# channable/alfred-margaret

Measured on AMD Instinct MI355X. Metric: GiB/s haystack bytes scanned (match-emitting runLower, 100k-needle automaton), higher is better.
Workload: dtype u8

## Files before the change

alfred-margaret_amd/csrc/am_kernels.hip:

```cpp
#include <hip/hip_runtime.h>

#include <atomic>
#include <cstdlib>
#include <type_traits>

#include "am_bounds.h"
#include "am_config.h"
#include "am_device.h"
#include "am_wave.h"

AM_BOUNDS_TU("am_kernels.hip")

namespace am {
namespace dev {


__global__ void k_hidx(const uint64_t* __restrict__ offsets, uint32_t n_hay, uint64_t total, uint32_t* __restrict__ hidx, uint64_t n_entries,
                       uint32_t* __restrict__ z0, uint64_t n0, uint32_t* __restrict__ z1, uint64_t n1)
{
    const uint64_t k = (uint64_t)blockIdx.x * blockDim.x + threadIdx.x;
    const uint64_t stride = (uint64_t)gridDim.x * blockDim.x;
    for (uint64_t i = k; i < n0; i += stride) z0[i] = 0u;
    for (uint64_t i = k; i < n1; i += stride) z1[i] = 0u;
    if (k >= n_entries) return;
    uint64_t p = k << kHidxShift;
    if (p > total - 1) p = total - 1;
    uint32_t lo = 0, hi = n_hay - 1;
    while (lo < hi) {
        const uint32_t mid = lo + (hi - lo + 1u) / 2u;
        if (offsets[mid] <= p) lo = mid; else hi = mid - 1u;
    }
    hidx[k] = lo;
}


constexpr int kSfThreads = 1024;
constexpr int kSfWaves = kSfThreads / 64;
constexpr int kSfLightThreads = 256;
constexpr uint64_t kSfLightChunks = 16;
constexpr int kSfQ1 = 128;
constexpr int kSfQ2 = 256;
constexpr uint32_t kSfMaxUnitChunks = 64;
constexpr uint32_t kSfWqIters = 2;
constexpr uint32_t kSfEpochChunks = 16;
constexpr int kSfStage = 1056;
constexpr uint32_t kSfMaskBytes = kBloomMasks * 4u;

template <bool IC, int MODE, int ILP, int LW, bool SHORT, bool DBG, int NT = kSfThreads, bool CHILDREN = false>
__global__ __launch_bounds__(NT) void k_sf(SfView s, BatchView b, ScanOut o, uint64_t n_chunks)
{
    constexpr int kSfThreads = NT, kSfWaves = NT / 64;
    constexpr bool kFlagMode = MODE == kModeAny || MODE == kModeIds;
    constexpr bool CH = CHILDREN, children = CHILDREN;
    constexpr uint32_t kEpoch = kFlagMode ? 4u : CH ? 8u : kSfEpochChunks;
    extern __shared__ __attribute__((aligned(16))) uint32_t lds[];
    const uint32_t words = 1u << s.bloom_log2_words;
    uint32_t* masks = lds;
    uint32_t* bloom = lds + kBloomMasks;
    uint8_t* stage_all = reinterpret_cast<uint8_t*>(bloom + words);
    uint16_t* q1_all = reinterpret_cast<uint16_t*>(stage_all + kSfWaves * kSfStage);
    uint16_t* q2_all = q1_all + kSfWaves * kSfQ1;

    for (uint32_t i = threadIdx.x; i < kBloomMasks; i += kSfThreads) masks[i] = bloom_mask_entry(i);
    for (uint32_t i = threadIdx.x; i < words; i += kSfThreads) bloom[i] = s.scan_bloom[i];
    __syncthreads();

    const uint32_t lane = threadIdx.x & 63u, wave = __builtin_amdgcn_readfirstlane(threadIdx.x >> 6);
    const uint32_t stage = kSfMaskBytes + 4u * words + wave * (uint32_t)kSfStage;
    const uint32_t q1 = kSfMaskBytes + 4u * words + (uint32_t)kSfWaves * kSfStage + wave * (uint32_t)(kSfQ1 * 2);
    const uint32_t q2 = kSfMaskBytes + 4u * words + (uint32_t)kSfWaves * (kSfStage + kSfQ1 * 2) + wave * (uint32_t)(kSfQ2 * 2);
    const uint32_t wq_cap = o.wq_cap;
    const uint32_t wq = kSfMaskBytes + 4u * words + (uint32_t)kSfWaves * (kSfStage + kSfQ1 * 2 + kSfQ2 * 2) + wave * (wq_cap * 64u);
    uint32_t wq_n = 0;
    (void)stage_all; (void)q1_all; (void)q2_all;
    const uint64_t n_waves = (uint64_t)gridDim.x * kSfWaves;
    const uint32_t log2_words = s.bloom_log2_words, tiers = s.tiers & ~kSfKeyFold;
    const uint32_t UC = o.unit_chunks;
    const uint64_t n_units = (n_chunks + UC - 1) / UC;
    uint64_t nval = 0;
    uint32_t q2_head = 0, q2_tail = 0;
    uint64_t unit_base_chunk = 0, epoch_base_chunk = 0;
    uint32_t unit_count = 0, unit_slots = 0, cur_block = kNone, first_block = kNone, grant_next = 0, grant_left = 0;
    bool pool_ok = true;

    const bool timing = DBG && o.dbg != nullptr;
    uint64_t t_filter = 0, t_compact = 0, t_probe = 0, t_resolve = 0, t_probe_pre = 0, t_mark = 0;
    uint64_t dbg_iters[8] = {0, 0, 0, 0, 0, 0, 0, 0};
    uint64_t t_r0 = 0, t_r1 = 0, t_r2 = 0, t_r3 = 0, n_batches = 0, n_cand = 0, n_probes = 0, n_defer = 0, n_found = 0;
    auto tick = [&](uint64_t& acc) { if (timing) { const uint64_t now = __builtin_amdgcn_s_memtime(); acc += now - t_mark; t_mark = now; } };

    uint32_t cnt_hay = kNone; uint64_t cnt_val = 0;
    auto flush_count = [&]() {
        if (cnt_hay != kNone && cnt_val && lane == 0) atomicAdd(reinterpret_cast<unsigned long long*>(o.hay_counts + cnt_hay), (unsigned long long)cnt_val);
        cnt_val = 0;
    };
    auto add_counts = [&](bool found, uint32_t hay, uint32_t vlen) {
        if (found) nval += vlen;
        const uint64_t fm = __ballot(found);
        if (!o.hay_counts || !fm) return;
        const uint32_t h0 = __shfl(hay, __ffsll((unsigned long long)fm) - 1, 64);
        if (__ballot(found && hay != h0) == 0) {
            const uint64_t sum = wave_sum_u64(found ? (uint64_t)vlen : 0ull);
            if (h0 != cnt_hay) { flush_count(); cnt_hay = h0; }
            cnt_val += sum;
        } else if (found) atomicAdd(reinterpret_cast<unsigned long long*>(o.hay_counts + hay), (unsigned long long)vlen);
    };
    auto walk_parked = [&]() {
        const uint32_t n = wq_n < 64u ? wq_n : 64u, base = wq_n - n;
        wq_n = base;
        const bool valid = lane < n;
        const uint32_t e = wq + (base + (valid ? lane : 0u)) * 64u;
        const u32x4_n a0 = *reinterpret_cast<const lds_u32x4_t*>((uintptr_t)e), a1 = *reinterpret_cast<const lds_u32x4_t*>((uintptr_t)(e + 16u)),
                      a2 = *reinterpret_cast<const lds_u32x4_t*>((uintptr_t)(e + 32u)), a3 = *reinterpret_cast<const lds_u32x4_t*>((uintptr_t)(e + 48u));
        uint64_t gpos[1] = {((uint64_t)a0.y << 32) | a0.x};
        uint32_t avail[1] = {a0.z}, depth[1] = {a1.x}, best_state[1] = {a1.y}, best_vlen[1] = {a1.z}, w2[1] = {a1.w}, node[1] = {kNone};
        const uint32_t slot = a0.w, hay = a3.z, prior = a1.y;
        SfNode rec[1] = {SfNode{0, 0, a2.x, a2.y, {a2.z, a2.w, a3.x, a3.y}}};
        bool go[1] = {valid}, have_rec[1] = {true};
        wave_lds_fence();
        uint32_t sel[1] = {a3.w};
        sf_resolve_walk<IC, 1>(s, b.text, gpos, avail, w2, go, node, rec, have_rec, depth, best_state, best_vlen, nullptr, 0xFFFFFFFFu, nullptr, sel);
        if (SHORT) {
            const bool vv[1] = {valid && !best_state[0]};
            uint32_t w[1] = {0}, dummy = 0;
            if (vv[0]) { load_suffix8(b.text, gpos[0], w[0], dummy); if (IC) w[0] = fold_dword(w[0]); }
            sf_resolve_short<1>(s, vv, avail, w, best_state, best_vlen);
        }
        const bool found = valid && best_state[0] != 0;
        if (timing) n_found += (uint32_t)__popcll(__ballot(found && prior == 0u));
        if (MODE == kModeCount) add_counts(found, hay, best_vlen[0]);
        else if (MODE == kModeEmit) {
            if (found && best_state[0] != prior && pool_ok) { AM_BOUNDS(slot < (uint64_t)o.n_blocks * kPoolBlock); o.pool[slot].state = best_state[0] - 1u; }
            unit_count += (uint32_t)__popcll(__ballot(found && prior == 0u));
        } else if (MODE == kModeAny && found) atomicOr(reinterpret_cast<uint32_t*>(o.flags) + (hay >> 2), 1u << (8u * (hay & 3u)));
    };

    constexpr int RN = 1;
    auto resolve_batch = [&](uint32_t nb, bool drain) {
        __builtin_amdgcn_s_setprio(3);
        if (timing) { const uint64_t now = __builtin_amdgcn_s_memtime(); t_r0 += now - t_mark; t_mark = now; n_batches++; }
        uint64_t gpos[RN];
        uint32_t w2[RN], avail[RN], best_state[RN], best_vlen[RN], depth[RN], hay[RN], slot[RN], sel[RN];
        SfNode rec[RN];
        bool parked[RN];
        uint64_t pm[RN];
#pragma unroll
        for (int k = 0; k < RN; k++) {
            gpos[k] = 0; w2[k] = avail[k] = best_state[k] = best_vlen[k] = depth[k] = hay[k] = slot[k] = 0;
            rec[k] = SfNode{0, 0, 0, 0, {0, 0, 0, 0}}; parked[k] = false; pm[k] = 0; sel[k] = kSelUnknown;
        }
        if (nb) {
            bool valid[RN];
            uint32_t hint[RN], hlo[RN], hhi[RN];
            uint64_t end_pos[RN];
#pragma unroll
            for (int k = 0; k < RN; k++) {
                valid[k] = 64u * k + lane < nb;
                const uint32_t item = valid[k] ? lds_read_u16(q2 + 2u * ((q2_head + 64u * k + lane) % kSfQ2)) : 0u;
                gpos[k] = (epoch_base_chunk + ((item >> 12) & (kEpoch - 1u))) * kSfChunk + (item & 1023u);
                hint[k] = ((item >> 10) & 3u) | ((CH && children) ? (item >> 13) & 4u : 0u);
                hlo[k] = hhi[k] = 0; end_pos[k] = 0;
                if (valid[k]) { hlo[k] = b.hidx[gpos[k] >> kHidxShift]; hhi[k] = b.hidx[(gpos[k] >> kHidxShift) + 1]; }
            }
            auto locate = [&]() {
#pragma unroll
                for (int k = 0; k < RN; k++) {
                    hay[k] = hlo[k];
                    uint64_t start = valid[k] ? b.offsets[hlo[k]] : 0;
                    if (valid[k] && hlo[k] != hhi[k]) { hay[k] = find_haystack(b, gpos[k]); start = b.offsets[hay[k]]; }
                    end_pos[k] = valid[k] ? gpos[k] - start + 1 : 0;
                }
            };
            uint32_t w[RN], node[RN], t16[RN][4];
            bool go[RN], have_rec[RN], found[RN];
            sf_resolve_head<IC, RN>(s, b.text, gpos, end_pos, valid, hint, locate, w, w2, avail, best_state, best_vlen, depth, go, node, rec, have_rec, t16, timing ? dbg_iters : nullptr);
            sf_resolve_walk<IC, RN>(s, b.text, gpos, avail, w2, go, node, rec, have_rec, depth, best_state, best_vlen, timing ? dbg_iters : nullptr, wq_cap ? o.wq_iters : 0xFFFFFFFFu, t16, sel);
#pragma unroll
            for (int k = 0; k < RN; k++) parked[k] = go[k] && valid[k];
            if (SHORT) {
                bool vv[RN];
#pragma unroll
                for (int k = 0; k < RN; k++) vv[k] = valid[k] && !parked[k];
                sf_resolve_short<RN>(s, vv, avail, w, best_state, best_vlen);
            }
#pragma unroll
            for (int k = 0; k < RN; k++) {
                found[k] = valid[k] && best_state[k] != 0;
                if (timing) n_found += (uint32_t)__popcll(__ballot(found[k]));
            }
            if (MODE == kModeCount) {
#pragma unroll
                for (int k = 0; k < RN; k++) add_counts(found[k] && !parked[k], hay[k], best_vlen[k]);
            } else if (MODE == kModeEmit && RN == 1) {
                const uint64_t take_mask = __ballot(found[0] || parked[0]);
                const uint32_t F = (uint32_t)__popcll(take_mask);
                if (F) {
                    const uint32_t r = unit_slots & (kPoolBlock - 1u);
                    const bool need_new = r == 0u || r + F > kPoolBlock;
                    uint32_t new_block = kNone;
                    if (need_new) {
                        if (grant_left == 0) {
                            uint32_t g = 0;
                            if (lane == 0) g = atomicAdd(o.pool_ctrl, kSfBlockGrant);
                            grant_next = __builtin_amdgcn_readfirstlane(g);
                            grant_left = kSfBlockGrant;
                        }
                        const uint32_t id = grant_next++;
                        grant_left--;
                        if (id >= o.n_blocks) { pool_ok = false; if (lane == 0) o.pool_ctrl[1] = 1u; }
                        else {
                            new_block = id;
                            if (lane == 0) { o.block_next[id] = kNone; if (cur_block != kNone) o.block_next[cur_block] = id; }
                            if (first_block == kNone) first_block = id;
                        }
                    }
                    if ((found[0] || parked[0]) && pool_ok) {
                        const uint32_t p = r + (uint32_t)__popcll(take_mask & ((1ull << lane) - 1ull));
                        slot[0] = (r != 0u && p < kPoolBlock) ? cur_block * kPoolBlock + p : new_block * kPoolBlock + (r != 0u ? p - kPoolBlock : p);
                        AM_BOUNDS(slot[0] < (uint64_t)o.n_blocks * kPoolBlock && hay[0] < b.n_hay);
                        o.pool[slot[0]] = Record{end_pos[0], hay[0], found[0] ? best_state[0] - 1u : kNone};
                    }
                    if (need_new && pool_ok) cur_block = new_block;
                    unit_slots += F;
                    unit_count += (uint32_t)__popcll(__ballot(found[0]));
                }
            } else if (MODE == kModeEmit) {
                uint64_t take[RN]; uint32_t before[RN], F = 0, n_found_recs = 0;
#pragma unroll
                for (int k = 0; k < RN; k++) {
                    take[k] = __ballot(found[k] || parked[k]); before[k] = F; F += (uint32_t)__popcll(take[k]);
                    n_found_recs += (uint32_t)__popcll(__ballot(found[k]));
                }
                if (F) {
                    const uint32_t s0 = unit_slots, have = (s0 + kPoolBlock - 1u) / kPoolBlock;
                    const uint32_t n_new = (s0 + F + kPoolBlock - 1u) / kPoolBlock - have;
                    const uint32_t prev_block = cur_block;
                    uint32_t ids[RN + 1];
#pragma unroll
                    for (int t = 0; t < RN + 1; t++) {
                        ids[t] = kNone;
                        if ((uint32_t)t < n_new) {
                            if (grant_left == 0) {
                                uint32_t g = 0;
                                if (lane == 0) g = atomicAdd(o.pool_ctrl, kSfBlockGrant);
                                grant_next = __builtin_amdgcn_readfirstlane(g);
                                grant_left = kSfBlockGrant;
                            }
                            const uint32_t id = grant_next++;
                            grant_left--;
                            if (id >= o.n_blocks) { pool_ok = false; if (lane == 0) o.pool_ctrl[1] = 1u; }
                            else if (pool_ok) {
                                ids[t] = id;
                                if (lane == 0) { o.block_next[id] = kNone; if (cur_block != kNone) o.block_next[cur_block] = id; }
                                if (first_block == kNone) first_block = id;
                                cur_block = id;
                            }
                        }
                    }
#pragma unroll
                    for (int k = 0; k < RN; k++) {
                        if ((found[k] || parked[k]) && pool_ok) {
                            const uint32_t si = s0 + before[k] + (uint32_t)__popcll(take[k] & ((1ull << lane) - 1ull));
                            const uint32_t q = si / kPoolBlock;
                            uint32_t blk = prev_block;
#pragma unroll
                            for (int t = 0; t < RN + 1; t++) if (q == have + (uint32_t)t) blk = ids[t];
                            slot[k] = blk * kPoolBlock + (si & (kPoolBlock - 1u));
                            AM_BOUNDS(slot[k] < (uint64_t)o.n_blocks * kPoolBlock && hay[k] < b.n_hay);
                            o.pool[slot[k]] = Record{end_pos[k], hay[k], found[k] ? best_state[k] - 1u : kNone};
                        }
                    }
                    unit_slots += F;
                    unit_count += n_found_recs;
                }
            } else if (MODE == kModeAny) {
#pragma unroll
                for (int k = 0; k < RN; k++) {
                    const uint64_t fm = __ballot(found[k]);
                    if (fm) {
                        const uint32_t h0 = __shfl(hay[k], __ffsll((unsigned long long)fm) - 1, 64);
                        const bool same = __ballot(found[k] && hay[k] != h0) == 0;
                        const bool mine = found[k] && (same ? lane == (uint32_t)__ffsll((unsigned long long)fm) - 1u : true);
                        if (mine) {
                            uint32_t* word = reinterpret_cast<uint32_t*>(o.flags) + (hay[k] >> 2);
                            const uint32_t bit = 1u << (8u * (hay[k] & 3u));
                            if (!(__atomic_load_n(word, __ATOMIC_RELAXED) & bit)) atomicOr(word, bit);
                        }
                    }
                }
            } else {
#pragma unroll
                for (int k = 0; k < RN; k++) {
                    if (found[k]) {
                        const uint32_t st = best_state[k] - 1u;
                        uint32_t* row = o.ids_bits + (uint64_t)hay[k] * o.ids_words;
                        for (uint64_t v = o.ids_vals_off[st], ve = o.ids_vals_off[st + 1]; v < ve; v++) {
                            const uint32_t id = o.ids_vals[v];
                            if (id >= o.ids_n) continue;
                            const uint32_t bit = 1u << (id & 31u);
                            if (row[id >> 5] & bit) continue;
                            if (!(atomicOr(row + (id >> 5), bit) & bit) && atomicSub(o.ids_missing + hay[k], 1u) == 1u)
                                atomicOr(reinterpret_cast<uint32_t*>(o.flags) + (hay[k] >> 2), 1u << (8u * (hay[k] & 3u)));
                        }
                    }
                }
            }
#pragma unroll
            for (int k = 0; k < RN; k++) pm[k] = __ballot(parked[k]);
        }
        uint64_t pm_any = 0;
#pragma unroll
        for (int k = 0; k < RN; k++) pm_any |= pm[k];
        if (pm_any || (drain && wq_n)) {
            int next_k = 0;
            for (;;) {
#pragma unroll
                for (int k = 0; k < RN; k++) {
                    if (next_k == k) {
                        const uint32_t n_park = (uint32_t)__popcll(pm[k]);
                        if (wq_n + n_park <= wq_cap) {
                            if (parked[k]) {
                                const uint32_t e = wq + (wq_n + (uint32_t)__popcll(pm[k] & ((1ull << lane) - 1ull))) * 64u;
                                AM_BOUNDS(e + 64u <= wq + wq_cap * 64u);
                                lds_write_u32x4(e, make_uint4((uint32_t)gpos[k], (uint32_t)(gpos[k] >> 32), avail[k], slot[k]));
                                lds_write_u32x4(e + 16u, make_uint4(depth[k], best_state[k], best_vlen[k], w2[k]));
                                lds_write_u32x4(e + 32u, make_uint4(rec[k].z, rec[k].w, rec[k].label[0], rec[k].label[1]));
                                lds_write_u32x4(e + 48u, make_uint4(rec[k].label[2], rec[k].label[3], hay[k], sel[k]));
                            }
                            wq_n += n_park;
                            wave_lds_fence();
                            next_k = k + 1;
                        }
                    }
                }
                if (next_k == RN && (drain ? wq_n == 0u : wq_n < 64u)) break;
                walk_parked();
                wave_lds_fence();
            }
        }
        if (timing) { const uint64_t now = __builtin_amdgcn_s_memtime(); t_r3 += now - t_mark; t_mark = now; }
        q2_head += nb;
        __builtin_amdgcn_s_setprio(2);
    };

    u32x2 p_a[2], p_b[2];
    uint32_t p_e[2] = {0, 0}, p_pos[2] = {0, 0};
    uint32_t p_k5[2] = {0, 0}, p_e5[2] = {0, 0};
    uint32_t p_ci = 0;
    bool pending = false, p_two = false;
    p_a[0] = p_a[1] = p_b[0] = p_b[1] = u32x2{0, 0};
    auto consume_round = [&]() {
        auto park = [&](bool defer, uint32_t hint, uint32_t pos) {
            const uint64_t m = __ballot(defer);
            AM_BOUNDS(q2_tail - q2_head + (uint32_t)__popcll(m) <= (uint32_t)kSfQ2);
            if (defer) lds_write_u16(q2 + 2u * ((q2_tail + (uint32_t)__popcll(m & ((1ull << lane) - 1ull))) % kSfQ2), (p_ci << 12) | ((hint & 3u) << 10) | (pos & 1023u) | (CH ? (hint & 4u) << 13 : 0u));
            q2_tail += (uint32_t)__popcll(m);
            if (timing) n_defer += (uint32_t)__popcll(m);
        };
        if (ILP == 2 || p_two) {
            bool valid[2], defer[2];
            uint32_t hint[2];
#pragma unroll
            for (int k = 0; k < 2; k++) valid[k] = (p_pos[k] & 0x8000u) != 0;
            sf_probe_decide<2>(s, p_a, p_b, p_e, valid, defer, hint);
            if (CH && children) {
                bool heavy[2];
                sf_probe_heavy<2>(s, p_a, p_b, p_e, defer, heavy);
                if (wave_any(heavy[0] || heavy[1])) sf_probe_children<2>(s, p_k5, p_e5, heavy, defer, hint);
            }
            park(defer[0], hint[0], p_pos[0]);
            park(defer[1], hint[1], p_pos[1]);
        } else {
            const u32x2 a1[1] = {p_a[0]}, b1[1] = {p_b[0]};
            const uint32_t e1[1] = {p_e[0]};
            const bool valid[1] = {(p_pos[0] & 0x8000u) != 0};
            bool defer[1]; uint32_t hint[1];
            sf_probe_decide<1>(s, a1, b1, e1, valid, defer, hint);
            if (CH && children) {
                bool heavy[1];
                sf_probe_heavy<1>(s, a1, b1, e1, defer, heavy);
                if (wave_any(heavy[0])) { const uint32_t k5[1] = {p_k5[0]}, e5[1] = {p_e5[0]}; sf_probe_children<1>(s, k5, e5, heavy, defer, hint); }
            }
            park(defer[0], hint[0], p_pos[0]);
        }
        pending = false;
    };

    auto fetch = [&](uint64_t cc, uint4& v) {
        const uint64_t p = cc * kSfChunk + lane * 16u;
        v = make_uint4(0, 0, 0, 0);
        if (cc < n_chunks && p < b.total) {
            typedef uint32_t u32x4_native __attribute__((ext_vector_type(4)));
            const u32x4_native* src = reinterpret_cast<const u32x4_native*>(b.text + p);
            const u32x4_native t = *src;
            v = make_uint4(t.x, t.y, t.z, t.w);
        }
    };
    auto fetch_before = [&](uint64_t cc, uint32_t& c3, uint32_t& c4) {
        uint2 t = make_uint2(0, 0);
        if (cc < n_chunks && cc > 0) {
            t = *reinterpret_cast<const uint2*>(b.text + cc * kSfChunk - 8);
            t.x = (uint32_t)__builtin_amdgcn_readfirstlane((int)t.x); t.y = (uint32_t)__builtin_amdgcn_readfirstlane((int)t.y);
        }
        c3 = IC ? fold_dword(t.x) : t.x; c4 = IC ? fold_dword(t.y) : t.y;
    };
    const uint64_t t_begin = timing ? __builtin_amdgcn_s_memtime() : 0;
    if (timing) t_mark = t_begin;
    uint64_t u = (uint64_t)blockIdx.x * kSfWaves + wave;
    uint64_t hs0 = 1, he0 = 0; uint32_t hay0 = 0;
    uint4 cur_v; uint32_t carry3, carry4;
    fetch(u * UC, cur_v);
    fetch_before(u * UC, carry3, carry4);
    asm volatile("" : "+v"(cur_v.x), "+v"(cur_v.y), "+v"(cur_v.z), "+v"(cur_v.w));

    uint32_t any_word = 0, any_hay = kNone, flagged_hay = kNone;

    uint64_t u_next = u;
    for (; u < n_units; u = u_next) {
        u_next = u + n_waves;
        if (o.next_unit && !kFlagMode) {
            uint32_t ticket = 0;
            if (lane == 0) ticket = atomicAdd(o.next_unit, 1u);
            u_next = n_waves + (uint32_t)__builtin_amdgcn_readfirstlane((int)ticket);
        }
        unit_base_chunk = u * UC;
        unit_count = 0; unit_slots = 0; cur_block = kNone; first_block = kNone;
        const uint32_t n_in_unit = (uint32_t)(unit_base_chunk + UC <= n_chunks ? UC : n_chunks - unit_base_chunk);
        if (kFlagMode && flagged_hay != kNone && hay0 == flagged_hay) {
            const uint64_t ub = unit_base_chunk * kSfChunk, ue0 = ub + (uint64_t)n_in_unit * kSfChunk, ue = ue0 < b.total ? ue0 : b.total;
            if (ub >= hs0 && he0 >= b.total) break;
            if (ub >= hs0 && ue <= he0) {
                fetch(u_next * UC, cur_v);
                fetch_before(u_next * UC, carry3, carry4);
                asm volatile("" : "+v"(cur_v.x), "+v"(cur_v.y), "+v"(cur_v.z), "+v"(cur_v.w));
                continue;
            }
        }
        bool jumped = false;
        for (uint32_t ci = 0; ci < n_in_unit; ci++) {
            const uint64_t c = unit_base_chunk + ci;
            if ((ci & (kEpoch - 1u)) == 0 && !jumped) epoch_base_chunk = c;
            uint4 next_v = make_uint4(0, 0, 0, 0);
            uint32_t next_c3 = 0, next_c4 = 0;
            const bool last_of_unit = ci + 1 >= n_in_unit;
            if (kFlagMode && any_hay != kNone) {
                const uint32_t seen = (uint32_t)__builtin_amdgcn_readfirstlane((int)any_word);
                if (((seen >> (8u * (any_hay & 3u))) & 0xFFu) != 0u) flagged_hay = any_hay;
                any_hay = kNone;
            }
            if (kFlagMode && last_of_unit) {
                if (flagged_hay != kNone && flagged_hay == hay0 && he0 >= b.total && unit_base_chunk * kSfChunk >= hs0) u_next = n_units;
                else if (o.next_unit) {
                    uint32_t ticket = 0;
                    if (lane == 0) ticket = atomicAdd(o.next_unit, 1u);
                    u_next = n_waves + (uint32_t)__builtin_amdgcn_readfirstlane((int)ticket);
                }
            }
            const bool next_skipped = kFlagMode && !last_of_unit && flagged_hay != kNone && flagged_hay == hay0 &&
                                      (c + 1) * kSfChunk >= hs0 && (c + 2) * kSfChunk <= he0;
            if (!next_skipped)
            fetch(!last_of_unit ? c + 1 : u_next * UC, next_v);
            if (last_of_unit) fetch_before(u_next * UC, next_c3, next_c4);

            const uint64_t c0 = c * kSfChunk;
            const uint64_t p0 = c0 + lane * 16u;
            if (c0 >= he0 || c0 < hs0) {
                hay0 = (uint32_t)__builtin_amdgcn_readfirstlane((int)b.hidx[c0 >> kHidxShift]);
                hs0 = uniform_u64(b.offsets[hay0]); he0 = uniform_u64(b.offsets[hay0 + 1]);
            }
            const bool single = (c0 + kSfChunk < b.total ? c0 + kSfChunk : b.total) <= he0;
            bool skip = false;
            if (kFlagMode) {
                skip = single && flagged_hay == hay0;
                if (skip && ci + 2 < n_in_unit) {
                    const uint64_t ue0 = (unit_base_chunk + n_in_unit) * kSfChunk;
                    if ((ue0 < b.total ? ue0 : b.total) <= he0) { ci = n_in_unit - 2u; jumped = true; }
                }
                if (!skip && (ci & 7u) == 0u) {
                    any_word = __hip_atomic_load(reinterpret_cast<const uint32_t*>(o.flags) + (hay0 >> 2), __ATOMIC_RELAXED, __HIP_MEMORY_SCOPE_AGENT);
                    any_hay = hay0;
                }
            }

            uint32_t d1 = cur_v.x, d2 = cur_v.y, d3 = cur_v.z, d4 = cur_v.w;
            if (IC) { d1 = fold_dword(d1); d2 = fold_dword(d2); d3 = fold_dword(d3); d4 = fold_dword(d4); }
            const uint32_t d0 = (uint32_t)__builtin_amdgcn_update_dpp((int)carry4, (int)d4, 0x138, 0xf, 0xf, false);
            const uint32_t f[5] = {bloom_key(d0, IC), bloom_key(d1, IC), bloom_key(d2, IC), bloom_key(d3, IC), bloom_key(d4, IC)};
            lds_write_u32x4(stage + 16u + lane * 16u, make_uint4(d1, d2, d3, d4));
            if (lane == 0) lds_write_u32x2(stage + 8u, make_uint2(carry3, carry4));
            if (!last_of_unit) {
                next_c3 = (uint32_t)__builtin_amdgcn_readlane((int)d3, 63);
                next_c4 = (uint32_t)__builtin_amdgcn_readlane((int)d4, 63);
            }
            __builtin_amdgcn_s_setprio(0);
            uint32_t cand = 0;
            if (!kFlagMode || !skip) {
                uint32_t h[16], v[16], m[16];
                const uint32_t sh_word = 32u - log2_words;
#pragma unroll
                for (int k = 0; k < 16; k++) {
                    const int j = k >> 2, sh = k & 3;
                    const uint32_t w = sh == 3 ? f[j + 1] : __builtin_amdgcn_alignbyte(f[j + 1], f[j], sh + 1);
                    h[k] = w * kBloomMul;
                }
#pragma unroll
                for (int k = 15; k >= 0; k--) {
                    if (LW) v[k] = lds_read_u32(kSfMaskBytes + ((h[k] >> (30 - LW)) & (((1u << LW) - 1u) << 2)));
                    else v[k] = lds_read_u32(kSfMaskBytes + ((h[k] >> sh_word) << 2));
                    m[k] = lds_read_u32(h[k] & ((kBloomMasks - 1u) << 2));
                }
                __builtin_amdgcn_sched_barrier(0);
#pragma unroll
                for (int k = 15; k >= 0; k--) {
                    const uint32_t mr = rotr32(m[k], scan_rot(h[k]));
                    cand = shift_in_eq(cand, v[k] & mr, mr);
                }
            }
            if (SHORT && (!kFlagMode || !skip)) {
#pragma unroll
                for (int k = 0; k < 16; k++) {
                    const int j = k >> 2, sh = k & 3;
                    const uint32_t w = sh == 3 ? f[j + 1] : __builtin_amdgcn_alignbyte(f[j + 1], f[j], sh + 1);
                    if (sf_filter_short<true>(bloom, log2_words, tiers, w, masks)) cand |= 1u << k;
                }
            }
            __builtin_amdgcn_s_setprio(2);
            if (p0 + 16 > b.total) cand &= p0 < b.total ? (1u << (uint32_t)(b.total - p0)) - 1u : 0u;
            if (timing) { asm volatile("" :: "v"(cand)); tick(t_filter); }

            for (bool first = true;; first = false) {
                const uint32_t n = __popc(cand);
                const uint32_t incl = wave_inclusive_sum(n, lane);
                const uint32_t total = wave_last_lane(incl);
                if (total == 0 && !(first && pending)) break;
                uint32_t idx = incl - n;
                while (cand && idx < (uint32_t)kSfQ1) {
                    const uint32_t k = __builtin_ctz(cand);
                    cand &= cand - 1u;
                    AM_BOUNDS(idx < (uint32_t)kSfQ1);
                    lds_write_u16(q1 + 2u * idx++, lane * 16u + k);
                }
                const uint32_t n_q1 = total < (uint32_t)kSfQ1 ? total : (uint32_t)kSfQ1;
                if (timing) n_cand += n_q1;
                wave_lds_fence();
                tick(t_compact);
                if (pending) {
                    consume_round();
                    wave_lds_fence();
                    tick(t_probe);
                    while (q2_tail - q2_head >= 64u * RN) { resolve_batch(64u * RN, false); wave_lds_fence(); }
                    tick(t_resolve);
                }
                if (n_q1) {
                    uint64_t avail[2] = {0, 0};
                    uint32_t w[2] = {0, 0}, nb[2] = {0, 0};
                    bool valid[2] = {false, false};
                    const bool two = ILP == 2 || n_q1 > 64u || o.two_always;
                    p_pos[1] = 0u;
#pragma unroll
                    for (int k = 0; k < 2; k++) {
                        if (k == 1 && !two) break;
                        const uint32_t e = 64u * k + lane;
                        valid[k] = e < n_q1;
                        const uint32_t pos = valid[k] ? lds_read_u16(q1 + 2u * e) : 0u;
                        if (CH && children) {
                            const uint32_t a = 10u + pos, sh = a & 3u;
                            const uint32_t sp = stage + (a & ~3u);
                            const uint32_t x0 = lds_read_u32(sp), x1 = lds_read_u32(sp + 4u), x2 = lds_read_u32(sp + 8u);
                            const uint32_t three = __builtin_amdgcn_alignbyte(x1, x0, sh) & 0xFFFFFFu;
                            const uint32_t nbs3 = (three >> 16) | (three & 0xFF00u) | ((three & 0xFFu) << 16);
                            nb[k] = nbs3 & 0xFFFFu;
                            w[k] = sh < 1u ? __builtin_amdgcn_alignbyte(x1, x0, 3u) : __builtin_amdgcn_alignbyte(x2, x1, sh - 1u);
                            t4_child_inputs(s, w[k], nbs3, p_k5[k], p_e5[k]);
                        } else {
                        const uint32_t a = 11u + pos, sh = a & 3u;
                        const uint32_t sp = stage + (a & ~3u);
                        const uint32_t x0 = lds_read_u32(sp), x1 = lds_read_u32(sp + 4u), x2 = lds_read_u32(sp + 8u);
                        const uint32_t two = __builtin_amdgcn_alignbyte(x1, x0, sh) & 0xFFFFu;
                        nb[k] = (two >> 8) | ((two & 0xFFu) << 8);
                        w[k] = sh < 2u ? __builtin_amdgcn_alignbyte(x1, x0, sh + 2u) : __builtin_amdgcn_alignbyte(x2, x1, sh - 2u);
                        }
                        const uint64_t gpos = c0 + pos;
                        avail[k] = gpos - hs0 + 1;
                        if (valid[k] && !single) avail[k] = gpos - b.offsets[find_haystack(b, gpos)] + 1;
                        p_pos[k] = valid[k] ? (pos | 0x8000u) : 0u;
                    }
                    if (two) sf_probe_issue<2>(s, w, nb, avail, valid, p_a, p_b, p_e);
                    else {
                        const uint32_t w1[1] = {w[0]}, nb1[1] = {nb[0]};
                        const uint64_t av1[1] = {avail[0]};
                        const bool v1[1] = {valid[0]};
                        u32x2 a1[1], b1[1]; uint32_t e1[1];
                        sf_probe_issue<1>(s, w1, nb1, av1, v1, a1, b1, e1);
                        p_a[0] = a1[0]; p_b[0] = b1[0]; p_e[0] = e1[0];
                    }
                    p_two = two;
                    p_ci = ci & (kEpoch - 1u);
                    pending = true;
                    if (timing) { n_probes++; tick(t_probe_pre); }
                }
                if (total <= (uint32_t)kSfQ1) break;
                wave_lds_fence();
            }
            cur_v = next_v; carry3 = next_c3; carry4 = next_c4;
            if ((ci & (kEpoch - 1u)) == kEpoch - 1u || last_of_unit) {
                if (pending) consume_round();
                wave_lds_fence();
                tick(t_compact);
                const bool walk_all = last_of_unit || kFlagMode;
                while (q2_tail != q2_head || (walk_all && wq_n)) {
                    const uint32_t left = q2_tail - q2_head, nb = left < 64u * RN ? left : 64u * RN;
                    resolve_batch(nb, walk_all && left == nb);
                }
                tick(t_resolve);
            }
        }
        if (MODE == kModeEmit && lane == 0) { o.unit_counts[u] = unit_count; o.unit_first[u] = first_block; o.unit_slots[u] = unit_slots; }
    }
    if (timing && lane == 0) {
        atomicAdd(reinterpret_cast<unsigned long long*>(o.dbg + 0), (unsigned long long)t_filter);
        atomicAdd(reinterpret_cast<unsigned long long*>(o.dbg + 1), (unsigned long long)t_compact);
        atomicAdd(reinterpret_cast<unsigned long long*>(o.dbg + 2), (unsigned long long)t_probe);
        atomicAdd(reinterpret_cast<unsigned long long*>(o.dbg + 3), (unsigned long long)t_resolve);
        atomicAdd(reinterpret_cast<unsigned long long*>(o.dbg + 4), 1ull);
        atomicAdd(reinterpret_cast<unsigned long long*>(o.dbg + 5), (unsigned long long)t_probe_pre);
        atomicAdd(reinterpret_cast<unsigned long long*>(o.dbg + 6), (unsigned long long)n_batches);
        atomicAdd(reinterpret_cast<unsigned long long*>(o.dbg + 7), (unsigned long long)t_r0);
        atomicAdd(reinterpret_cast<unsigned long long*>(o.dbg + 8), (unsigned long long)t_r1);
        atomicAdd(reinterpret_cast<unsigned long long*>(o.dbg + 9), (unsigned long long)t_r2);
        atomicAdd(reinterpret_cast<unsigned long long*>(o.dbg + 10), (unsigned long long)t_r3);
        for (int i = 0; i < 7; i++) atomicAdd(reinterpret_cast<unsigned long long*>(o.dbg + 16 + 2 * 8192 + i), (unsigned long long)dbg_iters[i]);
        atomicAdd(reinterpret_cast<unsigned long long*>(o.dbg + 11), (unsigned long long)n_cand);
        atomicAdd(reinterpret_cast<unsigned long long*>(o.dbg + 12), (unsigned long long)n_probes);
        atomicAdd(reinterpret_cast<unsigned long long*>(o.dbg + 13), (unsigned long long)n_defer);
        atomicAdd(reinterpret_cast<unsigned long long*>(o.dbg + 14), (unsigned long long)n_found);
        atomicMax(reinterpret_cast<unsigned long long*>(o.dbg + 15), (unsigned long long)(__builtin_amdgcn_s_memtime() - t_begin));
        const uint64_t gw = (uint64_t)blockIdx.x * kSfWaves + wave;
        if (gw < 8192) {
            uint32_t hw_id, xcc_id;
            asm volatile("s_getreg_b32 %0, hwreg(HW_REG_HW_ID)" : "=s"(hw_id));
            asm volatile("s_getreg_b32 %0, hwreg(HW_REG_XCC_ID)" : "=s"(xcc_id));
            o.dbg[16 + 2 * gw] = __builtin_amdgcn_s_memtime() - t_begin;
            o.dbg[17 + 2 * gw] = ((uint64_t)xcc_id << 32) | hw_id;
        }
    }

    if (MODE == kModeCount) {
        if (o.hay_counts) flush_count();
        nval = wave_sum_u64(nval);
        if (lane == 0 && nval) atomicAdd(reinterpret_cast<unsigned long long*>(o.total_values), (unsigned long long)nval);
    }
}

__global__ __launch_bounds__(256) void k_permute(ScanOut o, const uint64_t* __restrict__ unit_offsets, Record* __restrict__ out, uint64_t n_units)
{
    const uint64_t u = ((uint64_t)blockIdx.x * blockDim.x + threadIdx.x) >> 6;
    const uint32_t lane = threadIdx.x & 63u;
    if (u >= n_units) return;
    const uint32_t n = o.unit_slots[u];
    uint64_t at = unit_offsets[u];
    uint32_t blk = o.unit_first[u];
    const uint4* pool4 = reinterpret_cast<const uint4*>(o.pool);
    uint4* out4 = reinterpret_cast<uint4*>(out);
    for (uint32_t done = 0; done < n; done += kPoolBlock) {
        if (blk == kNone) break;
        uint4 r = make_uint4(0u, 0u, 0u, kNone);
        if (done + lane < n) r = pool4[(uint64_t)blk * kPoolBlock + lane];
        const uint64_t m = __ballot(r.w != kNone);
        if (r.w != kNone) out4[at + (uint32_t)__popcll(m & ((1ull << lane) - 1ull))] = r;
        at += (uint32_t)__popcll(m);
        blk = o.block_next[blk];
    }
}


hipError_t launch_hidx(const BatchView& b, uint32_t* hidx, uint64_t n_entries, hipStream_t st, uint32_t* z0, uint64_t n0, uint32_t* z1, uint64_t n1)
{
    const uint32_t blocks = (uint32_t)((n_entries + 255) / 256);
    hipLaunchKernelGGL(k_hidx, dim3(blocks), dim3(256), 0, st, b.offsets, b.n_hay, b.total, hidx, n_entries, z0, n0, z1, n1);
    return hipGetLastError();
}

uint64_t sf_chunks(const BatchView& b) { return (b.total + kSfChunk - 1) / kSfChunk; }

uint32_t sf_unit_chunks(const BatchView& b, int n_cu)
{
    const uint64_t n_chunks = sf_chunks(b), waves = (uint64_t)(n_cu > 0 ? n_cu : 1) * kSfWaves;
    const uint64_t per_wave = (n_chunks + waves - 1) / waves;
    const uint64_t k = (per_wave + kSfMaxUnitChunks - 1) / kSfMaxUnitChunks;
    if (k >= 4) return kSfMaxUnitChunks;
    const uint64_t uc = k <= 1 ? per_wave : (n_chunks + waves * k - 1) / (waves * k);
    return (uint32_t)(uc < 1 ? 1 : uc);
}

hipError_t launch_permute(const ScanOut& o, const uint64_t* unit_offsets, Record* out, uint64_t n_units, hipStream_t st)
{
    if (n_units == 0) return hipSuccess;
    const uint64_t blocks = (n_units * 64 + 255) / 256;
    hipLaunchKernelGGL(k_permute, dim3((uint32_t)blocks), dim3(256), 0, st, o, unit_offsets, out, n_units);
    return hipGetLastError();
}
uint64_t ac_units(const AcView& a, const BatchView& b) { return (b.total + a.chunk - 1) / a.chunk; }

static size_t sf_lds_bytes_w(const SfView& s, int waves) { return kSfMaskBytes + ((size_t)4 << s.bloom_log2_words) + (size_t)waves * (kSfStage + kSfQ1 * sizeof(uint16_t) + kSfQ2 * sizeof(uint16_t)); }
static uint32_t sf_wq_cap(const SfView& s, int waves)
{
    const size_t base = sf_lds_bytes_w(s, waves), limit = 160 * 1024;
    if (base >= limit) return 0;
    size_t cap = (limit - base) / ((size_t)waves * 64);
    if (cap > 128) cap = 128;
    return cap >= 64 ? (uint32_t)cap : 0u;
}
size_t sf_lds_bytes(const SfView& s) { return sf_lds_bytes_w(s, kSfWaves); }

constexpr uint32_t kSfVariantValid = 1u, kSfVariantIc = 2u, kSfVariantModeShift = 2, kSfVariantIlpShift = 4, kSfVariantShort = 1u << 6, kSfVariantDbg = 1u << 7,
                   kSfVariantLight = 1u << 8, kSfVariantChildren = 1u << 9, kSfVariantLwShift = 16;
static std::atomic<uint32_t> g_sf_last_variant{0};
uint32_t take_sf_last_variant() { return g_sf_last_variant.exchange(0, std::memory_order_relaxed); }

template <bool IC, int MODE, int ILP, int LW, bool SHORT, bool DBG = false, int NT = kSfThreads, bool CHILDREN = false>
static hipError_t launch_sf_v(const SfView& s, const BatchView& b, const ScanOut& o, int n_cu, hipStream_t st)
{
    constexpr int waves_per_wg = NT / 64;
    constexpr bool kFlagMode = MODE == kModeAny || MODE == kModeIds;
    const uint32_t wq_cap = kFlagMode ? 0u : sf_wq_cap(s, waves_per_wg);
    const size_t lds = sf_lds_bytes_w(s, waves_per_wg) + (size_t)waves_per_wg * wq_cap * 64;
    static bool attr_set = false;
    if (!attr_set) {
        if (hipFuncSetAttribute(reinterpret_cast<const void*>(&k_sf<IC, MODE, ILP, LW, SHORT, DBG, NT, CHILDREN>), hipFuncAttributeMaxDynamicSharedMemorySize, 160 * 1024) != hipSuccess)
            (void)hipGetLastError();
        attr_set = true;
    }
    const uint64_t n_chunks = sf_chunks(b);
    const int per_cu = NT == kSfThreads ? (lds <= 80 * 1024 ? 2 : 1) : 8;
    uint64_t blocks = (uint64_t)n_cu * per_cu;
    const uint64_t n_units = (n_chunks + o.unit_chunks - 1) / o.unit_chunks;
    const uint64_t need = (n_units + waves_per_wg - 1) / waves_per_wg;
    if (blocks > need) blocks = need;
    if (blocks == 0) return hipSuccess;
    g_sf_last_variant.store(kSfVariantValid | (IC ? kSfVariantIc : 0u) | ((uint32_t)MODE << kSfVariantModeShift) | ((uint32_t)ILP << kSfVariantIlpShift) | (SHORT ? kSfVariantShort : 0u) |
                            (DBG ? kSfVariantDbg : 0u) | (NT == kSfLightThreads ? kSfVariantLight : 0u) | (CHILDREN ? kSfVariantChildren : 0u) | ((uint32_t)LW << kSfVariantLwShift),
                            std::memory_order_relaxed);
    ScanOut oo = o;
    oo.wq_cap = wq_cap;
    oo.wq_iters = kSfWqIters;
    if (n_units <= blocks * waves_per_wg) oo.next_unit = nullptr;
    hipLaunchKernelGGL((k_sf<IC, MODE, ILP, LW, SHORT, DBG, NT, CHILDREN>), dim3((uint32_t)blocks), dim3(NT), lds, st, s, b, oo, n_chunks);
    return hipGetLastError();
}

static uint64_t* g_sf_dbg = nullptr;
hipError_t read_sf_wave_records(uint64_t* out, size_t n_waves)
{
    if (!g_sf_dbg) return hipErrorInvalidValue;
    if (n_waves == 0) { hipError_t e = hipMemcpy(out, g_sf_dbg + 16 + 2 * 8192, 64, hipMemcpyDeviceToHost); if (e == hipSuccess) e = hipMemset(g_sf_dbg + 16 + 2 * 8192, 0, 64); return e; }
    return hipMemcpy(out, g_sf_dbg + 16, 16 * (n_waves < 8192 ? n_waves : 8192), hipMemcpyDeviceToHost);
}

hipError_t read_sf_phase_cycles(uint64_t* out5)
{
    for (int i = 0; i < 16; i++) out5[i] = 0;
    if (!g_sf_dbg) return hipSuccess;
    hipError_t e = hipMemcpy(out5, g_sf_dbg, 128, hipMemcpyDeviceToHost);
    if (e == hipSuccess) e = hipMemset(g_sf_dbg, 0, 128);
    return e;
}

template <bool IC, int MODE>
static hipError_t launch_sf_t(const SfView& s, const BatchView& b, const ScanOut& o, int n_cu, hipStream_t st)
{
    const bool lw15 = s.bloom_log2_words == 15;
    constexpr bool kFlagMode = MODE == kModeAny || MODE == kModeIds;
    if constexpr (MODE == kModeIds) {
        if (sf_chunks(b) <= kSfLightChunks)
            return (s.tiers & 7u) ? launch_sf_v<IC, MODE, 2, 0, true, false, kSfLightThreads>(s, b, o, n_cu, st) : launch_sf_v<IC, MODE, 2, 0, false, false, kSfLightThreads>(s, b, o, n_cu, st);
        return (s.tiers & 7u) ? launch_sf_v<IC, MODE, 2, 0, true>(s, b, o, n_cu, st) : launch_sf_v<IC, MODE, 2, 0, false>(s, b, o, n_cu, st);
    } else {
    if (o.dbg && !kFlagMode) {
        if (!lw15) return launch_sf_v<IC, MODE, 2, 0, true, true>(s, b, o, n_cu, st);
        return (s.tiers & 7u) ? launch_sf_v<IC, MODE, 2, 15, true, true>(s, b, o, n_cu, st) : launch_sf_v<IC, MODE, 2, 15, false, true>(s, b, o, n_cu, st);
    }
    if (sf_chunks(b) <= kSfLightChunks)
        return (s.tiers & 7u) ? launch_sf_v<IC, MODE, 2, 0, true, false, kSfLightThreads>(s, b, o, n_cu, st) : launch_sf_v<IC, MODE, 2, 0, false, false, kSfLightThreads>(s, b, o, n_cu, st);
    if (!lw15 && s.t4_children && !(s.tiers & 7u) && !kFlagMode) return launch_sf_v<IC, MODE, 2, 0, false, false, kSfThreads, true>(s, b, o, n_cu, st);
    const bool few = s.tier_log2_cap[3] <= 15u;
    if (s.tiers & 7u) {
        if (few) return lw15 ? launch_sf_v<IC, MODE, 1, 15, true>(s, b, o, n_cu, st) : launch_sf_v<IC, MODE, 1, 0, true>(s, b, o, n_cu, st);
        return lw15 ? launch_sf_v<IC, MODE, 2, 15, true>(s, b, o, n_cu, st) : launch_sf_v<IC, MODE, 2, 0, true>(s, b, o, n_cu, st);
    }
    if (few) return lw15 ? launch_sf_v<IC, MODE, 1, 15, false>(s, b, o, n_cu, st) : launch_sf_v<IC, MODE, 1, 0, false>(s, b, o, n_cu, st);
    return lw15 ? launch_sf_v<IC, MODE, 2, 15, false>(s, b, o, n_cu, st) : launch_sf_v<IC, MODE, 2, 0, false>(s, b, o, n_cu, st);
    }
}

hipError_t launch_sf(bool ic, int mode, const SfView& s, const BatchView& b, const ScanOut& o_in, int n_cu, hipStream_t st)
{
    ScanOut o = o_in;
    o.two_always = 0;
    static uint64_t* dbg = nullptr;
    if (cfg::on(cfg::kSfTrace)) {
        if (!dbg) { if (hipMalloc((void**)&dbg, 256 + 16 * 8192) != hipSuccess) dbg = nullptr; else (void)hipMemset(dbg, 0, 256 + 16 * 8192); }
        o.dbg = dbg;
        g_sf_dbg = dbg;
    }
    if (ic) {
        if (mode == kModeCount) return launch_sf_t<true, kModeCount>(s, b, o, n_cu, st);
        if (mode == kModeEmit) return launch_sf_t<true, kModeEmit>(s, b, o, n_cu, st);
        if (mode == kModeIds) return launch_sf_t<true, kModeIds>(s, b, o, n_cu, st);
        return launch_sf_t<true, kModeAny>(s, b, o, n_cu, st);
    }
    if (mode == kModeCount) return launch_sf_t<false, kModeCount>(s, b, o, n_cu, st);
    if (mode == kModeEmit) return launch_sf_t<false, kModeEmit>(s, b, o, n_cu, st);
    if (mode == kModeIds) return launch_sf_t<false, kModeIds>(s, b, o, n_cu, st);
    return launch_sf_t<false, kModeAny>(s, b, o, n_cu, st);
}

}
}
```

alfred-margaret_amd/csrc/am_wave.h:

```cpp
#pragma once
#include <hip/hip_runtime.h>
#include <stdint.h>

namespace am {
namespace dev {


__device__ __forceinline__ uint32_t lane_id() { return __builtin_amdgcn_mbcnt_hi(~0u, __builtin_amdgcn_mbcnt_lo(~0u, 0u)); }

__device__ __forceinline__ uint32_t wave_inclusive_sum(uint32_t x, uint32_t )
{
    x += (uint32_t)__builtin_amdgcn_update_dpp(0, (int)x, 0x111, 0xf, 0xf, false);
    x += (uint32_t)__builtin_amdgcn_update_dpp(0, (int)x, 0x112, 0xf, 0xf, false);
    x += (uint32_t)__builtin_amdgcn_update_dpp(0, (int)x, 0x114, 0xf, 0xf, false);
    x += (uint32_t)__builtin_amdgcn_update_dpp(0, (int)x, 0x118, 0xf, 0xf, false);
    x += (uint32_t)__builtin_amdgcn_update_dpp(0, (int)x, 0x142, 0xa, 0xf, false);
    x += (uint32_t)__builtin_amdgcn_update_dpp(0, (int)x, 0x143, 0xc, 0xf, false);
    return x;
}

__device__ __forceinline__ uint32_t wave_last_lane(uint32_t x) { return (uint32_t)__builtin_amdgcn_readlane((int)x, 63); }

__device__ __forceinline__ uint32_t shift_in_eq(uint32_t acc, uint32_t a, uint32_t b)
{
    asm("v_cmp_eq_u32 vcc, %1, %2\n\tv_addc_co_u32 %0, vcc, %0, %0, vcc" : "+v"(acc) : "v"(a), "v"(b) : "vcc");
    return acc;
}

__device__ __forceinline__ uint64_t uniform_u64(uint64_t x)
{
    const uint32_t lo = (uint32_t)__builtin_amdgcn_readfirstlane((int)(uint32_t)x), hi = (uint32_t)__builtin_amdgcn_readfirstlane((int)(uint32_t)(x >> 32));
    return ((uint64_t)hi << 32) | lo;
}

__device__ __forceinline__ uint64_t wave_sum_u64(uint64_t x)
{
#pragma unroll
    for (int d = 32; d > 0; d >>= 1) x += __shfl_down(x, d, 64);
    return x;
}

__device__ __forceinline__ void wave_lds_fence()
{
    __builtin_amdgcn_fence(__ATOMIC_RELEASE, "wavefront");
    __builtin_amdgcn_wave_barrier();
    __builtin_amdgcn_fence(__ATOMIC_ACQUIRE, "wavefront");
}

typedef __attribute__((address_space(3))) uint32_t lds_u32_t;
typedef __attribute__((address_space(3))) uint16_t lds_u16_t;
typedef uint32_t u32x2_n __attribute__((ext_vector_type(2)));
typedef uint32_t u32x4_n __attribute__((ext_vector_type(4)));
typedef __attribute__((address_space(3))) u32x2_n lds_u32x2_t;
typedef __attribute__((address_space(3))) u32x4_n lds_u32x4_t;
__device__ __forceinline__ uint32_t lds_read_u32(uint32_t byte_addr) { return *reinterpret_cast<const lds_u32_t*>((uintptr_t)byte_addr); }
__device__ __forceinline__ uint32_t lds_read_u16(uint32_t byte_addr) { return *reinterpret_cast<const lds_u16_t*>((uintptr_t)byte_addr); }
__device__ __forceinline__ void lds_write_u16(uint32_t byte_addr, uint32_t v) { *reinterpret_cast<lds_u16_t*>((uintptr_t)byte_addr) = (uint16_t)v; }
__device__ __forceinline__ void lds_write_u32x2(uint32_t byte_addr, uint2 v) { u32x2_n t; t.x = v.x; t.y = v.y; *reinterpret_cast<lds_u32x2_t*>((uintptr_t)byte_addr) = t; }
__device__ __forceinline__ void lds_write_u32x4(uint32_t byte_addr, uint4 v) { u32x4_n t; t.x = v.x; t.y = v.y; t.z = v.z; t.w = v.w; *reinterpret_cast<lds_u32x4_t*>((uintptr_t)byte_addr) = t; }

__device__ __forceinline__ uint64_t skip_code_points_backwards(const uint8_t* hay, uint64_t end_pos, uint32_t n)
{
    int64_t index = (int64_t)end_pos - 1;
    for (;;) {
        if (index >= 0 && (hay[index] & 0xC0) == 0x80) { index--; continue; }
        if (index < 0) return 0;
        if (n == 0) return (uint64_t)index;
        index--; n--;
    }
}

}
}
```

Measured before the change: 1098.

## Reload kernargs in resolve paths and hoist per-chunk bounds checks to chunk indices

Inside the resolve and parked-walk lambdas, the SfView and ScanOut structs are reloaded from the kernarg segment so they do not stay live in SGPRs/VGPRs across the main scan loop, relieving register pressure. Haystack boundary tests are precomputed once per unit as chunk indices (he_ci, single_ci, tail_ci), which replaces per-chunk 64-bit compares with 32-bit index compares. Interior chunks use an unguarded fetch, and the tail mask is applied only on the last chunk. When ILP==2 and the total candidate count fits the queue, a queue-append loop without the bound check is used. The risks are that the KArgs layout must exactly match the real kernel argument order, and that the index bracketing must reproduce the old boundary semantics.

```diff
diff --git a/alfred-margaret_amd/csrc/am_kernels.hip b/alfred-margaret_amd/csrc/am_kernels.hip
--- a/alfred-margaret_amd/csrc/am_kernels.hip
+++ b/alfred-margaret_amd/csrc/am_kernels.hip
@@ -105,7 +105,10 @@
             cnt_val += sum;
         } else if (found) atomicAdd(reinterpret_cast<unsigned long long*>(o.hay_counts + hay), (unsigned long long)vlen);
     };
+    struct KArgs { SfView s; BatchView b; ScanOut o; uint64_t n_chunks; };
     auto walk_parked = [&]() {
+        const SfView s = kernarg_reload<SfView>(offsetof(KArgs, s));
+        const ScanOut o = kernarg_reload<ScanOut>(offsetof(KArgs, o));
         const uint32_t n = wq_n < 64u ? wq_n : 64u, base = wq_n - n;
         wq_n = base;
         const bool valid = lane < n;
@@ -137,6 +140,8 @@
 
     constexpr int RN = 1;
     auto resolve_batch = [&](uint32_t nb, bool drain) {
+        const SfView s = kernarg_reload<SfView>(offsetof(KArgs, s));
+        const ScanOut o = kernarg_reload<ScanOut>(offsetof(KArgs, o));
         __builtin_amdgcn_s_setprio(3);
         if (timing) { const uint64_t now = __builtin_amdgcn_s_memtime(); t_r0 += now - t_mark; t_mark = now; n_batches++; }
         uint64_t gpos[RN];
@@ -396,6 +401,11 @@
             v = make_uint4(t.x, t.y, t.z, t.w);
         }
     };
+    auto fetch_whole = [&](uint64_t cc, uint4& v) {
+        typedef uint32_t u32x4_native __attribute__((ext_vector_type(4)));
+        const u32x4_native t = *reinterpret_cast<const u32x4_native*>(b.text + cc * kSfChunk + lane * 16u);
+        v = make_uint4(t.x, t.y, t.z, t.w);
+    };
     auto fetch_before = [&](uint64_t cc, uint32_t& c3, uint32_t& c4) {
         uint2 t = make_uint2(0, 0);
         if (cc < n_chunks && cc > 0) {
@@ -415,6 +425,15 @@
 
     uint32_t any_word = 0, any_hay = kNone, flagged_hay = kNone;
 
+    uint32_t he_ci = 0, single_ci = 0, n_whole = 0, tail_ci = kNone;
+    auto bracket_ci = [&](uint64_t at) {
+        he_ci = 0; single_ci = 0;
+        if (at >= hs0 && at < he0) {
+            const uint64_t d = he0 - unit_base_chunk * kSfChunk, up = (d + kSfChunk - 1) / kSfChunk, down = d / kSfChunk;
+            he_ci = up < kNone ? (uint32_t)up : kNone;
+            single_ci = he0 >= b.total || down >= kNone ? kNone : (uint32_t)down;
+        }
+    };
     uint64_t u_next = u;
     for (; u < n_units; u = u_next) {
         u_next = u + n_waves;
@@ -436,6 +455,10 @@
                 continue;
             }
         }
+        tail_ci = unit_base_chunk + n_in_unit >= n_chunks ? n_in_unit - 1u : kNone;
+        n_whole = n_in_unit - 1u;
+        if (tail_ci != kNone && n_whole) n_whole--;
+        bracket_ci(unit_base_chunk * kSfChunk);
         bool jumped = false;
         for (uint32_t ci = 0; ci < n_in_unit; ci++) {
             const uint64_t c = unit_base_chunk + ci;
@@ -458,17 +481,20 @@
             }
             const bool next_skipped = kFlagMode && !last_of_unit && flagged_hay != kNone && flagged_hay == hay0 &&
                                       (c + 1) * kSfChunk >= hs0 && (c + 2) * kSfChunk <= he0;
-            if (!next_skipped)
-            fetch(!last_of_unit ? c + 1 : u_next * UC, next_v);
+            if (!next_skipped) {
+                if (ci < n_whole) fetch_whole(c + 1, next_v);
+                else fetch(!last_of_unit ? c + 1 : u_next * UC, next_v);
+            }
             if (last_of_unit) fetch_before(u_next * UC, next_c3, next_c4);
 
             const uint64_t c0 = c * kSfChunk;
             const uint64_t p0 = c0 + lane * 16u;
-            if (c0 >= he0 || c0 < hs0) {
+            if (ci >= he_ci) {
                 hay0 = (uint32_t)__builtin_amdgcn_readfirstlane((int)b.hidx[c0 >> kHidxShift]);
                 hs0 = uniform_u64(b.offsets[hay0]); he0 = uniform_u64(b.offsets[hay0 + 1]);
-            }
-            const bool single = (c0 + kSfChunk < b.total ? c0 + kSfChunk : b.total) <= he0;
+                bracket_ci(c0);
+            }
+            const bool single = ci < single_ci;
             bool skip = false;
             if (kFlagMode) {
                 skip = single && flagged_hay == hay0;
@@ -525,6 +551,7 @@
                 }
             }
             __builtin_amdgcn_s_setprio(2);
+            if (ci == tail_ci)
             if (p0 + 16 > b.total) cand &= p0 < b.total ? (1u << (uint32_t)(b.total - p0)) - 1u : 0u;
             if (timing) { asm volatile("" :: "v"(cand)); tick(t_filter); }
 
@@ -534,6 +561,14 @@
                 const uint32_t total = wave_last_lane(incl);
                 if (total == 0 && !(first && pending)) break;
                 uint32_t idx = incl - n;
+                if (ILP == 2 && total <= (uint32_t)kSfQ1) {
+                    while (cand) {
+                        const uint32_t k = __builtin_ctz(cand);
+                        cand &= cand - 1u;
+                        AM_BOUNDS(idx < (uint32_t)kSfQ1);
+                        lds_write_u16(q1 + 2u * idx++, lane * 16u + k);
+                    }
+                } else
                 while (cand && idx < (uint32_t)kSfQ1) {
                     const uint32_t k = __builtin_ctz(cand);
                     cand &= cand - 1u;
diff --git a/alfred-margaret_amd/csrc/am_wave.h b/alfred-margaret_amd/csrc/am_wave.h
--- a/alfred-margaret_amd/csrc/am_wave.h
+++ b/alfred-margaret_amd/csrc/am_wave.h
@@ -31,6 +31,18 @@
 {
     const uint32_t lo = (uint32_t)__builtin_amdgcn_readfirstlane((int)(uint32_t)x), hi = (uint32_t)__builtin_amdgcn_readfirstlane((int)(uint32_t)(x >> 32));
     return ((uint64_t)hi << 32) | lo;
+}
+
+template <class T>
+__device__ __forceinline__ T kernarg_reload(uint32_t offset)
+{
+    typedef const __attribute__((address_space(4))) char* kernarg_bytes;
+    kernarg_bytes p = (kernarg_bytes)__builtin_amdgcn_kernarg_segment_ptr();
+    asm volatile("" : "+s"(p));
+    typedef const __attribute__((address_space(4))) T* kernarg_t;
+    T out;
+    __builtin_memcpy(&out, (kernarg_t)(p + offset), sizeof(T));
+    return out;
 }
 
 __device__ __forceinline__ uint64_t wave_sum_u64(uint64_t x)
```

After: 1120, median of 6. 2.0% higher.
